# tokkiwa/FlashGMM

Hardware: AMD Instinct MI355X
Metric: encode+decode Mpixels/s (Kodak, K=4 N=192) + GMM-CDF HBM GB/s vs roofline (higher is better)
Workload: dtype f32; 1 GPU; kodak24; schedule=codec, images_per_gpu=24, K=4, approx_mode=polya, param_dtype=f32, coded_symbols_per_gpu=6223104, streams_per_gpu=48, one_device_rehearsal=False

## Files before the change

### flashgmm_amd/csrc/fgmm_capi.cpp

```cpp
#include <sched.h>

#include <string>

#include "fgmm_ctx.h"

using namespace fgmm;

namespace fgmm {

static thread_local char t_err[512] = "";
char *last_error_buffer(size_t *cap) {
  if (cap) *cap = sizeof t_err;
  return t_err;
}
int fail(int code, const char *fmt, ...) {
  va_list ap;
  va_start(ap, fmt);
  vsnprintf(t_err, sizeof t_err, fmt, ap);
  va_end(ap);
  return code;
}

}

// ... 123 lines not shown
  const char *name;
  int64_t fgmm_ctx::Opts::*field;
  int64_t lo, hi;
  const char *env;
};
const OptName kOpts[] = {
    {"pieces", &fgmm_ctx::Opts::pieces, 0, kMaxPieces, "FGMM_PIECES"},
    {"dec_first", &fgmm_ctx::Opts::dec_first, 1, 1 << 20, "FGMM_DEC_FIRST"},
    {"tab_cap_e", &fgmm_ctx::Opts::tab_cap_e, 256, 32768, "FGMM_TAB_CAP_E"},
    {"stage_max_mb", &fgmm_ctx::Opts::stage_max_mb, 0, 1 << 30, "FGMM_STAGE_MAX_MB"},
    {"trace", &fgmm_ctx::Opts::trace, 0, 2, "FGMM_TRACE"},
    {"enc_vec", &fgmm_ctx::Opts::enc_vec, 0, 8, "FGMM_VEC"},
    {"enc_linear", &fgmm_ctx::Opts::enc_linear, 0, 1, nullptr},
    {"ef_rows", &fgmm_ctx::Opts::ef_rows, 0, 2, "FGMM_EF_ROWS"},
    {"ef_min", &fgmm_ctx::Opts::ef_min, kTabEfMin, 1 << 20, "FGMM_EF_MIN_ROWS"},
    {"enc_ways", &fgmm_ctx::Opts::enc_ways, 0, kMaxEncWays, "FGMM_ENC_WAYS"},
    {"ckpt_decode", &fgmm_ctx::Opts::ckpt_decode, 0, 2, "FGMM_CKPT_DECODE"},
    {"spin_lat", &fgmm_ctx::Opts::spin_lat, -1, 1ll << 40, "FGMM_SPIN_LAT"},
    {"gpu_decode", &fgmm_ctx::Opts::gpu_decode, 0, 2, "FGMM_GPU_DECODE"},
    {"enc_segs", &fgmm_ctx::Opts::enc_segs, 0, 2, "FGMM_ENC_SEGS"},
    {"scatter_rounds", &fgmm_ctx::Opts::scatter_rounds, 0, 1, nullptr},
};
}

namespace {
double cgroup_cpu_quota() {
  double best = -1.0;
  auto take = [&best](double q) {
    if (q > 0 && (best < 0 || q < best)) best = q;
  };
// ... 727 lines not shown
  hd->meta = reinterpret_cast<uint32_t *>(ctx->d_ws + 1024);
  dev::Stream s = (dev::Stream)stream;
  DEV_TRY(dev::copy_async(ctx->d_ws, hd, sizeof *hd, dev::kH2D, s));
  DEV_TRY(dev::memset_async(ctx->d_ws + 1024, 0, meta_bytes, s));
  LAUNCH_TRY(launch_symtab(reinterpret_cast<const EncDesc *>(ctx->d_ws), 1, 1, n, n, false, mode, enc_vec4_ok(*hd, false) ? 4 : 1, false, false, s));
  DEV_TRY(dev::stream_sync(s));
  return FGMM_OK;
}

int fgmm_build_cdftab_hip(fgmm_ctx *ctx, void *stream, const float *scales, const float *means,
                          const float *weights, int64_t n, int64_t stride_n, int64_t stride_k, int mode,
                          int32_t max_bs, int flags, uint32_t *hdr, uint8_t *pool, uint64_t pool_cap,
                          uint64_t *pool_used) {
  if (!ctx || n < 0 || !mode_ok(mode) || !pool_used) return fail(FGMM_ERR_INVALID, "bad argument");
  if (max_bs < 0 || max_bs > FGMM_MAX_BS_H4) return fail(FGMM_ERR_UNSUPPORTED, "max_bs %d outside [0, %d] (4-byte headers)", max_bs, FGMM_MAX_BS_H4);
  std::lock_guard<std::mutex> lock(ctx->mu);
  DeviceGuard g(ctx->device);
  const int32_t tiles = (int32_t)((n + 255) / 256);
  const size_t o_bsum = 2048, o_boff = o_bsum + align_up(sizeof(uint32_t) * (size_t)tiles + 64, 256);
  int rc;
  if ((rc = ctx->ensure_device(o_boff + sizeof(uint64_t) * (size_t)tiles + 64)) || (rc = ctx->ensure_host(4096))) return rc;
  dev::Stream s = (dev::Stream)stream;
  DecDesc *hd = reinterpret_cast<DecDesc *>(ctx->h_ws);
  memset(hd, 0, sizeof *hd);
  hd->scales = scales;
  hd->means = means;
  hd->weights = weights;
  hd->stride_k = stride_k;
  hd->stride_p = stride_n;
  hd->hw = n;
// ... 42 lines not shown
  dev::Stream s = (dev::Stream)stream;
  DecDesc *hd = reinterpret_cast<DecDesc *>(ctx->h_ws);
  memset(hd, 0, sizeof *hd);
  hd->scales = scales;
  hd->means = means;
  hd->weights = weights;
  hd->stride_k = stride_k;
  hd->stride_p = stride_n;
  hd->hw = n;
  hd->n = n;
  hd->n_ch = 1;
  hd->max_bs = max_bs;
  hd->prune = (flags & FGMM_TAB_NO_PRUNE) ? 0 : 1;
  hd->clamp = (flags & FGMM_TAB_CLAMP) ? 1 : 0;
  hd->hdr_form = tab_hdr_form(max_bs);
  hd->ef_min = (flags & FGMM_TAB_RAW_ROWS) ? kTabNoEf : kTabEfMin;
  hd->tl = tl;
  hd->blk_begin = 0;
  hd->blk_end = (int32_t)nblk;
  hd->hdr_out = hdr;
  hd->blkoff_out = blk_off;
  hd->rows = rows;
  hd->rows_cap = rows_cap;
  hd->counters = reinterpret_cast<unsigned long long *>(ctx->d_ws + 1024);
  hd->count_edges = 1;
  unsigned long long cn[kTabCounters] = {};
  DEV_TRY(dev::copy_async(ctx->d_ws, hd, sizeof *hd, dev::kH2D, s));
  DEV_TRY(dev::memset_async(ctx->d_ws + 1024, 0, kCounterBytes, s));
  if (n) LAUNCH_TRY(launch_tab(reinterpret_cast<const DecDesc *>(ctx->d_ws), 1, (int)nblk, tl, cap_e, mode, (flags & FGMM_TAB_CLAMP) != 0, false, s));
  DEV_TRY(dev::copy_async(cn, ctx->d_ws + 1024, sizeof cn, dev::kD2H, s));
  DEV_TRY(dev::stream_sync(s));
// ... 63 lines not shown
```

### flashgmm_amd/csrc/fgmm_ctx.h

```cpp
#pragma once
#include <math.h>
#include <pthread.h>
#include <sched.h>
#include <stdarg.h>
#include <stdio.h>
#include <stdlib.h>
#include <string.h>

#include <algorithm>
#include <atomic>
#include <chrono>
#include <condition_variable>
#include <functional>
#include <mutex>
#include <queue>
#include <string>
#include <thread>
#include <vector>

#include "../../include/flashgmm_amd.h"
#include "fgmm_device.h"
#include "fgmm_internal.h"

namespace fgmm {
// ... 267 lines not shown
  std::mutex mu;
  fgmm::Pool *pool = nullptr;
  fgmm::WorkerCpus worker_cpus;
  fgmm::Pool *dec_pool = nullptr;
  fgmm::Pool *decoders() const { return dec_pool ? dec_pool : pool; }
  char *d_ws = nullptr;
  size_t d_cap = 0;
  char *h_ws = nullptr;
  size_t h_cap = 0;
  std::vector<fgmm::dev::Event> events;
  std::vector<fgmm::dev::Event> sleep_events;
  fgmm::dev::Stream copy_stream = nullptr;
  fgmm::dev::Stream aux_stream = nullptr;
  struct Opts {
    int64_t pieces = 0, dec_first = 2, tab_cap_e = fgmm::kTabCapE, stage_max_mb = 0, trace = 0, enc_vec = 0, enc_linear = 1, ef_rows = 0,
            ef_min = fgmm::kTabEfDefault, enc_ways = 0, ckpt_decode = 0, spin_lat = 400000, gpu_decode = 0, enc_segs = 1, scatter_rounds = 1;
  } opt;
  struct Chunk {
    char *p;
    size_t cap, used;
  };
  std::vector<Chunk> chunks;
  void chunks_reset() {
    for (auto &c : chunks) c.used = 0;
  }
  int chunk_alloc(size_t bytes, char **out);
  char *d_stage = nullptr;
  size_t d_stage_cap = 0;
  int ensure_stage(size_t bytes);
  size_t stage_budget() const;
  int ensure_streams();
// ... 103 lines not shown
```

### flashgmm_amd/csrc/fgmm_decode.cpp

```cpp
#include <array>

#include "fgmm_ctx.h"

namespace fgmm {
namespace {

struct Part {
  int item;
  int64_t blk_begin, blk_end;
  size_t o_hdr, o_blkoff;
  int piece;
};
struct Unit {
  std::vector<Part> parts;
  size_t fixed = 0, rows_cap = 0;
  size_t o_stage = 0;
  char *d_range = nullptr;
};
struct Key {
  int unit, item, seg;
  bool operator>(const Key &o) const { return unit != o.unit ? unit > o.unit : (item != o.item ? item > o.item : seg > o.seg); }
};

constexpr int kLaunchAhead = 3;

struct DecodeCall {
  fgmm_ctx *ctx;
  dev::Stream stream;
  std::vector<DecItem> &items;
  const int mode, count;
  Trace tr;
  int cap_e = kTabCapE, np = 1, decoders = 1;
  bool clamped = false, f16 = false, spin = false;
  uint32_t ef_min = kTabNoEf;
  int64_t streams_of_work = 0;
  bool lead_small = false;
  double lead_cum[kMaxPieces + 1] = {0};
  std::vector<int> fast, generic;
  std::vector<Unit> units;
  int n_units = 0;
  Arena ar;
  size_t o_descs = 0, o_scat = 0, o_counters = 0, upload_bytes = 0, stage_total = 0, n_parts = 0;
  std::vector<size_t> unit_desc0;
  int n_round = 0, M_round = 0;
  int64_t hw_round = 0;
  bool dead_round = false;
  dev::Event *ev_kernel = nullptr, *ev_counters = nullptr, *ev_landed = nullptr;
  TempDevice temp;
  int launched = 0;
// ... 20 lines not shown
    if (ctx->opt.tab_cap_e == kTabCapE)
      for (const DecItem &it : items)
        if (!tab_tl(it.max_bs, cap_e) && tab_tl(it.max_bs, kTabCapEWide)) {
          cap_e = kTabCapEWide;
          break;
        }
    clamped = items[0].clamp != 0;
    f16 = items[0].prm.dtype == FGMM_F16;
    const bool use_ckpt = ctx->opt.ckpt_decode == 1 || (ctx->opt.ckpt_decode == 0 && count < std::max(ctx->decoders()->size(), 1));
    for (auto &it : items) {
      if (!use_ckpt) it.ckpt = nullptr, it.n_ckpt = 0;
      streams_of_work += it.ckpt && it.n_ckpt > 0 ? it.n_ckpt + 1 : 1;
    }
    decoders = (int)std::min<int64_t>(std::max(ctx->decoders()->size(), 1), streams_of_work);
    ef_min = ctx->opt.ef_rows == 1 || (ctx->opt.ef_rows == 0 && decoders >= 10) ? (uint32_t)ctx->opt.ef_min : kTabNoEf;
    return FGMM_OK;
  }

  int plan_items() {
    for (int i = 0; i < count; ++i) {
      DecItem &it = items[i];
      if (it.max_bs < 0 || it.max_bs > FGMM_MAX_BS) return fail(FGMM_ERR_UNSUPPORTED, "max_bs_value %d outside [0, %d]", it.max_bs, FGMM_MAX_BS);
      it.n_ch = 0;
      for (int c = 0; c < it.M; ++c) it.n_ch += it.zero_bitmap ? (it.zero_bitmap[c] != 0) : 1;
      it.n = (int64_t)it.n_ch * it.hw;
      it.o_list = ar.take(sizeof(int32_t) * std::max(it.n_ch, 1), 16);
      it.o_rank = ar.take(sizeof(int32_t) * std::max(it.M, 1), 16);
      it.hdr_form = tab_hdr_form(it.max_bs);
      it.ef_min = ef_min;
      it.tl = tab_tl(it.max_bs, cap_e);
      it.nblk = it.tl ? (it.n + it.tl - 1) / it.tl : 0;
      if (it.nblk > 0x7FFFFFFFll) it.tl = 0, it.nblk = 0;
      (it.tl ? fast : generic).push_back(i);
    }
    return FGMM_OK;
  }

  void plan_pieces() {
    np = (int)std::min<int64_t>(std::max<int64_t>(ctx->opt.pieces, 1), kMaxPieces);
    int64_t lat = 0, lat_max = 0;
    for (int i : fast) lat += items[i].n, lat_max = std::max(lat_max, items[i].n);
    if (ctx->opt.pieces > 0) return;
    np = 8;
    while (np < kAutoPiecesMax && (int64_t)np * (np + 1) / 2 * 4096 < lat_max) ++np;
    if (lat < 65536) np = 1;
    if (decoders == 1 && np > 1) {
      lead_small = true;
// ... 141 lines not shown
    d.scales = it.prm.scales;
    d.means = it.prm.means;
    d.weights = it.prm.weights;
    d.stride_k = it.prm.stride_k;
    d.stride_c = it.prm.stride_c;
    d.stride_p = it.stride_p;
    d.hw = it.hw;
    d.n = it.n;
    d.chan_list = reinterpret_cast<const int32_t *>(ctx->d_ws + it.o_list);
    d.n_ch = it.n_ch;
    d.max_bs = it.max_bs;
    d.clamp = it.clamp;
    d.logits = (it.prm.flags & FGMM_PARAMS_LOGITS) ? 1 : 0;
    d.prune = 1;
    d.hdr_form = it.hdr_form;
    d.ef_min = ef_min;
    d.tl = it.tl;
    d.count_edges = ctx->profiling ? 1 : 0;
    return d;
  }
  void fill_unit_descs(int u) {
    const Unit &un = units[(size_t)u];
    DecDesc *hd = reinterpret_cast<DecDesc *>(ctx->h_ws + o_descs);
    for (size_t k = 0; k < un.parts.size(); ++k) {
      const Part &p = un.parts[k];
      DecDesc &d = hd[unit_desc0[(size_t)u] + k];
      d = base_desc(items[p.item]);
      d.blk_begin = (int32_t)p.blk_begin;
      d.blk_end = (int32_t)p.blk_end;
      d.hdr_out = un.d_range + p.o_hdr;
      d.blkoff_out = reinterpret_cast<uint32_t *>(un.d_range + p.o_blkoff);
// ... 526 lines not shown
```

### flashgmm_amd/csrc/fgmm_internal.h

```cpp
#pragma once
#include <stddef.h>
#include <stdint.h>

#include "../../include/flashgmm_amd.h"

#if defined(__HIPCC__)
#define FGMM_HD __host__ __device__
#else
#define FGMM_HD
#endif

namespace fgmm {


struct EncDesc {
  const float *y;
  const int32_t *sym;
  const void *scales, *means, *weights;
  int64_t stride_k, stride_c, stride_p;
  int64_t hw;
  int32_t M;
  int32_t clamp;
  int32_t logits;
  uint32_t meta_slots;
// ... 120 lines not shown
FGMM_HD static inline uint32_t tab_hdr_cnt(uint32_t h) { return (h >> 16) & 0x7FFFu; }
FGMM_HD static inline uint32_t tab_hdr_nonmono(uint32_t h) { return h >> 31; }
FGMM_HD static inline unsigned long long tab_hdr8_pack(int32_t a, uint32_t cnt, uint32_t nonmono) {
  return (unsigned long long)(uint32_t)a | ((unsigned long long)((cnt & 0x7FFFFFFFu) | (nonmono << 31)) << 32);
}
constexpr uint32_t kTabNoEf = 0x7FFFFFFFu;
FGMM_HD static inline bool tab_row_is_ef(uint32_t cnt, uint32_t nonmono, uint32_t ef_min) { return cnt >= ef_min && !nonmono; }
constexpr uint32_t kTabEf12Max = 48;
FGMM_HD static inline uint32_t tab_ef_l(uint32_t cnt) { return cnt <= kTabEf12Max ? 12u : 8u; }
FGMM_HD static inline uint32_t tab_ef_hb(uint32_t cnt, uint32_t l) { return cnt + (65536u >> l); }
FGMM_HD static inline uint32_t tab_ef_lb(uint32_t cnt, uint32_t l) { return (tab_ef_hb(cnt, l) + 7u) & ~7u; }
FGMM_HD static inline unsigned long long tab_ef_bits(uint32_t cnt, uint32_t l) { return (unsigned long long)cnt * l + tab_ef_lb(cnt, l); }
FGMM_HD static inline unsigned long long tab_row_bytes(uint32_t cnt, uint32_t nonmono, uint32_t ef_min) {
  return tab_row_is_ef(cnt, nonmono, ef_min) ? 2ull * ((tab_ef_bits(cnt, tab_ef_l(cnt)) + 15ull) >> 4) : 2ull * (unsigned long long)cnt;
}
FGMM_HD static inline bool tab_hdr_fits16(int32_t max_bs) { return 2 * (int64_t)max_bs + 2 <= 254; }
FGMM_HD static inline int tab_hdr_form(int32_t max_bs) { return tab_hdr_fits16(max_bs) ? 2 : (max_bs <= 16382 ? 4 : 8); }
constexpr int kTabCapE = 12288;
constexpr int kTabCapEWide = 16384;
constexpr int kTabMaxTl = 256;
FGMM_HD static inline int tab_tl(int32_t max_bs, int cap_e) {
  const int64_t W = 2 * (int64_t)max_bs + 2;
  const int64_t t = (cap_e / W) & ~15ll;
  return t >= 16 ? (int)(t > kTabMaxTl ? kTabMaxTl : t) : 0;
}

int launch_quant_stats(const EncDesc *d_descs, int count, int M_max, void *stream);
int launch_symtab(const EncDesc *d_descs, int count, int M_max, int64_t hw_max, int64_t n_max, bool linear, int mode, int vec,
                  bool clamped, bool f16, void *stream);
int launch_cdf_pair(const int32_t *v, const float *scales, const float *means, const float *weights, int64_t n,
// ... 86 lines not shown
```

### flashgmm_amd/csrc/fgmm_rans.cpp

```cpp
#include <immintrin.h>
#include <stdlib.h>
#include <string.h>

#include <cmath>
#include <mutex>
#include <vector>

#include "../../include/flashgmm_amd.h"
#include "fgmm_internal.h"

namespace fgmm {

namespace {

constexpr uint64_t kRansL = 1ull << 31;
constexpr uint32_t kPrec = 16;
constexpr uint32_t kMaxCdf = 65535;
constexpr uint32_t kBypassBits = 4;
constexpr uint32_t kMaxBypassVal = 15;

struct Rcp {
  uint64_t rcp;
  uint32_t shift;
  uint32_t bias_add;
// ... 494 lines not shown
      const int64_t rem = (int64_t)nbits - 64 * (int64_t)w;
      if (rem < 64) m &= (1ull << rem) - 1ull;
      if (m) break;
      if (__builtin_expect(++w >= r.words(), 0)) return -1;
      m = r[w];
    }
    const int32_t pos = w * 64 + (int32_t)__builtin_ctzll(m);
    e1 = ((uint32_t)(pos - j) << r.l) | r.low(j);
  }
  *jout = j;
  *start = e0;
  *freq = (e1 - e0) & 0xFFFFu;
  return 1;
}

}

int TabDecoder::begin(const uint8_t *enc, size_t enc_len, const TabView *view, int64_t n_, int32_t max_bs_, int32_t *out_) {
  tv = view;
  n = n_;
  max_bs = max_bs_;
  out = out_;
  i = 0;
  next_piece = 0;
  rc = FGMM_OK;
  copy = nullptr;
  scratch = nullptr;
  scratch_cap = 0;
  if (n < 0 || !enc || (n > 0 && (!out || !tv || !tv->piece || tv->npiece < 1))) return rc = FGMM_ERR_INVALID;
  if (tv && tv->hdr_form != 2 && tv->hdr_form != 4 && tv->hdr_form != 8) return rc = FGMM_ERR_INVALID;
// ... 97 lines not shown
        uint32_t h;
        memcpy(&h, rowp, 4);
        rowp += 4;
        cnt = tab_hdr_cnt(h);
        nonmono = tab_hdr_nonmono(h);
      }
    } else if (hdr_form == 4) {
      const uint32_t h = static_cast<const uint32_t *>(pc->hdr)[li];
      cnt = tab_hdr_cnt(h);
      nonmono = tab_hdr_nonmono(h);
    } else {
      const uint64_t h = static_cast<const uint64_t *>(pc->hdr)[li];
      cnt = (int64_t)((h >> 32) & 0x7FFFFFFFu);
      nonmono = (uint32_t)(h >> 63);
    }
    const uint64_t rbytes = tab_row_bytes((uint32_t)cnt, nonmono, ef_min);
    if (cnt < 1 || (uint64_t)(rows_end - rowp) < rbytes) { rc = FGMM_ERR_INVALID; return; }
    rowp += rbytes;
    ++i;
  }
  inline bool active() const { return rc == FGMM_OK && i < i_end; }
  void finish() {
    td->x = dec.x;
    td->ptr = dec.ptr;
    td->i = i;
    if (rc != FGMM_OK) td->rc = rc;
  }

  inline void open_block() {
    b_end = i + tl < i_end ? i + tl : i_end;
    if (pc->blk_off) {
      rowp = pc->rows + 4 * (size_t)pc->blk_off[blk];
      if (__builtin_expect(rowp > rows_end, 0)) {
        rc = FGMM_ERR_INVALID;
        return;
      }
      if (b_end < i_end) {
        const uint8_t *nx = pc->rows + 4 * (size_t)pc->blk_off[blk + 1];
        if (nx + FGMM_PREFETCH_AHEAD <= rows_end)
          for (int q = 0; q < FGMM_PREFETCH_AHEAD; q += 64) __builtin_prefetch(nx + q);
      }
    }
    ++blk;
  }

  __attribute__((always_inline)) inline void step() {
    if (__builtin_expect(i == b_end, 0)) {
      open_block();
      if (rc != FGMM_OK) return;
    }
    __builtin_prefetch(rowp + FGMM_PREFETCH_AHEAD);
    __builtin_prefetch(rowp + FGMM_PREFETCH_AHEAD + 64);
    int64_t a;
    int64_t cnt;
    uint32_t nonmono;
    const int64_t li = i - i_beg;
    if (hdr_form == 2) {
      const uint32_t c = static_cast<const uint16_t *>(pc->hdr)[li];
      a = (int64_t)(c & 0xFFu) - max_bs;
      cnt = c >> 8;
      nonmono = 0;
      if (__builtin_expect(cnt == kHdr2Escape, 0)) {
        if (rows_end - rowp < 4) { rc = FGMM_ERR_INVALID; return; }
        uint32_t h;
        memcpy(&h, rowp, 4);
        rowp += 4;
        a = tab_hdr_a(h);
        cnt = tab_hdr_cnt(h);
        nonmono = tab_hdr_nonmono(h);
      }
    } else if (hdr_form == 4) {
      const uint32_t h = static_cast<const uint32_t *>(pc->hdr)[li];
      a = tab_hdr_a(h);
      cnt = tab_hdr_cnt(h);
      nonmono = tab_hdr_nonmono(h);
    } else {
      const uint64_t h = static_cast<const uint64_t *>(pc->hdr)[li];
      a = (int32_t)(uint32_t)h;
      cnt = (int64_t)((h >> 32) & 0x7FFFFFFFu);
      nonmono = (uint32_t)(h >> 63);
    }
    if (__builtin_expect(cnt < 1 || a < -(int64_t)max_bs || a + max_bs + cnt > W, 0)) { rc = FGMM_ERR_INVALID; return; }
    const bool is_ef = tab_row_is_ef((uint32_t)cnt, nonmono, ef_min);
    const uint64_t rbytes = tab_row_bytes((uint32_t)cnt, nonmono, ef_min);
    if (__builtin_expect((uint64_t)(rows_end - rowp) < rbytes, 0)) { rc = FGMM_ERR_INVALID; return; }
    const bool zero_before = a > -(int64_t)max_bs;
    const uint8_t *row_bytes = rowp;
    rowp += rbytes;

    const uint32_t cf = (uint32_t)(dec.x & 0xFFFFu);
    int32_t value;
    if (__builtin_expect(cf == kMaxCdf, 0)) {
      value = dec.bypass();
    } else {
      uint32_t start = 0, freq = 0;
      bool done = false;
      if (!is_ef) {
        const uint16_t *row = reinterpret_cast<const uint16_t *>(row_bytes);
        if (__builtin_expect(!nonmono, 1)) {
          const int32_t j = upper_bound_u16(row, (int32_t)cnt, cf);
          if (__builtin_expect(j >= 1 && j < cnt, 1)) {
            start = row[j - 1];
            freq = (uint32_t)(row[j] - start) & 0xFFFFu;
            value = (int32_t)(a + j - 1);
            done = true;
          } else if (j == 0 && zero_before) {
            start = 0;
            freq = row[0];
            value = (int32_t)(a - 1);
            done = true;
          }
        }
// ... 9 lines not shown
          rc = FGMM_ERR_INVALID;
          return;
        } else {
          value = expand_and_bisect(r, a, cf, &start, &freq);
          if (rc != FGMM_OK) return;
        }
      }
      if (__builtin_expect(freq == 0, 0)) { rc = FGMM_ERR_INVALID; return; }
      dec.advance(start, freq);
    }
    td->out[i] = value;
    if (__builtin_expect(dec.underrun, 0)) { rc = FGMM_ERR_STREAM; return; }
    ++i;
  }

  __attribute__((noinline)) int32_t expand_and_bisect(const EfRow &r, int64_t a, uint32_t cf, uint32_t *start, uint32_t *freq) {
    const int32_t cnt = r.cnt;
    if ((size_t)cnt > td->scratch_cap) {
      free(td->scratch);
      td->scratch_cap = (size_t)cnt + 64;
      td->scratch = (uint16_t *)malloc(td->scratch_cap * sizeof(uint16_t));
      if (!td->scratch) {
        td->scratch_cap = 0;
        rc = FGMM_ERR_NOMEM;
        return 0;
      }
    }
    for (int32_t q = 0; q < cnt; ++q) {
      const int32_t pos = ef_select1(r, (uint32_t)q);
      if (pos < q) {
        rc = FGMM_ERR_INVALID;
        return 0;
      }
      td->scratch[q] = (uint16_t)((((uint32_t)(pos - q)) << r.l) | r.low(q));
    }
    return bisect_reference(Row{td->scratch, (int32_t)a, cnt}, cf, max_bs, start, freq);
  }
};

}

int TabDecoder::piece(int k) {
  PieceRun r;
  if (!r.begin(*this, k)) return r.rc;
  while (r.active()) r.step();
  r.finish();
  return rc;
}

int TabDecoder::segment(int64_t lo, int64_t hi, uint64_t x0, uint64_t pos0, uint64_t *x1, uint64_t *pos1) {
  if (rc != FGMM_OK) return rc;
  if (!tv || lo < 0 || hi > n || lo > hi || pos0 > (uint64_t)(end_ - base_)) return rc = FGMM_ERR_INVALID;
  x = x0;
  ptr = base_ + pos0;
  i = lo;
  int k = 0;
  while (k < tv->npiece && tv->piece[k].end <= lo) ++k;
  for (; i < hi && k < tv->npiece && rc == FGMM_OK; ++k) {
    PieceRun r;
    if (!r.begin_at(*this, k, hi)) {
      if (r.rc != FGMM_OK) rc = r.rc;
      break;
    }
    while (r.active()) r.step();
    r.finish();
  }
  if (rc == FGMM_OK && i < hi) rc = FGMM_ERR_INVALID;
  *x1 = x;
  *pos1 = (uint64_t)(ptr - base_);
  return rc;
}

int TabDecoder::finish() {
  if (rc == FGMM_OK && i < n) rc = FGMM_ERR_INVALID;
  free(copy);
  free(scratch);
  copy = nullptr;
  scratch = nullptr;
  return rc;
// ... 218 lines not shown
                                 size_t *out_len, fgmm_ckpt *ckpt_out) {
  if (stride < 0 || (stride & (stride - 1))) return FGMM_ERR_INVALID;
  return fgmm::rans_encode_symtab_ckpt(packed, symbols_or_null, n, -1, out, out_len, stride, ckpt_out);
}
int fgmm_rans_decode_tab_ckpt(const uint8_t *encoded, size_t encoded_len, const void *hdr, int hdr_form, const uint32_t *blk_off,
                              int32_t tl, const uint8_t *rows, uint64_t rows_len, int64_t n, int32_t max_bs, int flags,
                              const fgmm_ckpt *ckpt, int64_t n_ckpt, int64_t stride, int32_t *out_symbols, int32_t *verified_out) {
  if (verified_out) *verified_out = 0;
  if (!ckpt || n_ckpt == 0 || !blk_off || stride <= 0 || (stride & (stride - 1)) || n_ckpt != fgmm_ckpt_count(n, stride))
    return fgmm_rans_decode_tab(encoded, encoded_len, hdr, hdr_form, blk_off, tl, rows, rows_len, n, max_bs, flags, out_symbols);
  if (n > 0 && (!hdr || !rows)) return FGMM_ERR_INVALID;
  if (max_bs < 0 || max_bs > FGMM_MAX_BS || tl < 1) return FGMM_ERR_INVALID;
  if (hdr_form == 2 && !fgmm::tab_hdr_fits16(max_bs)) return FGMM_ERR_INVALID;
  if (hdr_form == 4 && max_bs > FGMM_MAX_BS_H4) return FGMM_ERR_INVALID;
  const fgmm::TabPiece pc{hdr, blk_off, rows, (size_t)rows_len, n};
  const fgmm::TabView tv{(flags & FGMM_TAB_RAW_ROWS) ? fgmm::kTabNoEf : fgmm::kTabEfMin, hdr_form, tl, 1, &pc, nullptr, nullptr};
  bool ok = true;
  int hard = FGMM_OK;
  fgmm::TabDecoder td;
  int rc = td.begin(encoded, encoded_len, &tv, n, max_bs, out_symbols);
  if (rc != FGMM_OK) {
    td.finish();
    return rc;
  }
  const uint64_t x_head = td.x;
  for (int64_t sgm = 0; sgm <= n_ckpt && ok; ++sgm) {
    const int64_t lo = sgm * stride, hi = sgm == n_ckpt ? n : (sgm + 1) * stride;
    const uint64_t x0 = sgm ? ckpt[sgm - 1].x : x_head, pos0 = sgm ? ckpt[sgm - 1].pos : 0;
    uint64_t x1 = 0, pos1 = 0;
    rc = td.segment(lo, hi, x0, pos0, &x1, &pos1);
    td.rc = FGMM_OK;
// ... 48 lines not shown
  for (int k = 0; k < ways; ++k) {
    syms[k] = symbols_or_null ? symbols_or_null[k] : nullptr;
    nb[k] = -1;
    out[k] = nullptr;
    o[k] = &out[k];
    l[k] = &out_len[k];
  }
  return fgmm::rans_encode_symtab_ways(ways, packed, syms, n, nb, o, l);
}

int fgmm_rans_decode_cdftab(const uint8_t *encoded, size_t encoded_len, const uint32_t *hdr, const uint8_t *pool,
                            uint64_t pool_len, int64_t n, int32_t max_bs, int flags, int32_t *out_symbols) {
  if (n > 0 && (!hdr || !pool)) return FGMM_ERR_INVALID;
  if (max_bs < 0 || max_bs > FGMM_MAX_BS_H4) return FGMM_ERR_UNSUPPORTED;
  const fgmm::TabPiece pc{hdr, nullptr, pool, (size_t)pool_len, n};
  const fgmm::TabView tv{(flags & FGMM_TAB_RAW_ROWS) ? fgmm::kTabNoEf : fgmm::kTabEfMin, 4, 0, 1, &pc, nullptr, nullptr};
  return fgmm::rans_decode_tab(encoded, encoded_len, tv, n, max_bs, out_symbols);
}

int fgmm_rans_decode_tab(const uint8_t *encoded, size_t encoded_len, const void *hdr, int hdr_form, const uint32_t *blk_off,
                         int32_t tl, const uint8_t *rows, uint64_t rows_len, int64_t n, int32_t max_bs, int flags,
                         int32_t *out_symbols) {
  if (n > 0 && (!hdr || !rows)) return FGMM_ERR_INVALID;
  if (max_bs < 0 || max_bs > FGMM_MAX_BS || (blk_off && tl < 1)) return FGMM_ERR_INVALID;
  if (hdr_form == 2 && !fgmm::tab_hdr_fits16(max_bs)) return FGMM_ERR_INVALID;
  if (hdr_form == 4 && max_bs > FGMM_MAX_BS_H4) return FGMM_ERR_INVALID;
  const fgmm::TabPiece pc{hdr, blk_off, rows, (size_t)rows_len, n};
  const fgmm::TabView tv{(flags & FGMM_TAB_RAW_ROWS) ? fgmm::kTabNoEf : fgmm::kTabEfMin, hdr_form, tl, 1, &pc, nullptr, nullptr};
  return fgmm::rans_decode_tab(encoded, encoded_len, tv, n, max_bs, out_symbols);
}

void fgmm_free(void *p) { free(p); }

struct fgmm_symbuf {
  fgmm::SymBuf sb;
};
struct fgmm_decstream {
  fgmm::DecStream ds;
};

int fgmm_symbuf_create(fgmm_symbuf **out) {
  if (!out) return FGMM_ERR_INVALID;
  *out = new (std::nothrow) fgmm_symbuf;
// ... 60 lines not shown
```

### flashgmm_amd/csrc/fgmm_tab.hip

```cpp
#include <algorithm>

#include "fgmm_dev.h"

namespace fgmm {

template <int MODE, bool CLAMPED, typename PT> struct TabLatent {
  float mu[4], sg[4], pi[4], rs[4];
  int max_bs;

  __device__ __forceinline__ void load(const DecDesc &d, int c, int64_t p) {
    const int64_t base = (int64_t)c * d.stride_c + p * d.stride_p;
#pragma unroll
    for (int k = 0; k < 4; ++k) {
      const float s = ld1<PT>(d.scales, base + k * d.stride_k);
      sg[k] = CLAMPED ? clamp_scale(s) : s;
      rs[k] = CLAMPED ? rcp_refined(sg[k]) : 0.0f;
      mu[k] = ld1<PT>(d.means, base + k * d.stride_k);
      pi[k] = ld1<PT>(d.weights, base + k * d.stride_k);
    }
    if (d.logits) softmax4(pi);
    max_bs = d.max_bs;
  }
  __device__ __forceinline__ uint32_t edge(int j) const {
    const float x = (float)(j - max_bs) - 0.5f;
// ... 429 lines not shown
      for (int q = 0; q < 8; ++q) v[q] = e32[(k >> 1) + q];
#pragma unroll
      for (int q = 0; q < 8; ++q) {
        ts.step(j_lo + k + 2 * q, v[q] & 0xFFFFu);
        ts.step(j_lo + k + 2 * q + 1, v[q] >> 16);
      }
    }
    for (; k < len; ++k) ts.step(j_lo + k, e[k]);
    int a_idx;
    uint32_t cnt;
    ts.finish(j_hi, W, S.tsat[tid], a_idx, cnt);
    const uint32_t nm = ts.nonmono ? 1u : 0u;
    S.meta[tid] = (uint32_t)a_idx | (cnt << 16);
    if (nm) S.flags[tid] |= 2;
    bytes = (uint32_t)tab_row_bytes(cnt, nm, d.ef_min);
    const int64_t li = (int64_t)(b - d.blk_begin) * tl + tid;
    if (d.hdr_form == 2) {
      const uint32_t c8 = nm ? kHdr2Escape : cnt;
      static_cast<uint16_t *>(d.hdr_out)[li] = (uint16_t)((uint32_t)a_idx | (c8 << 8));
      if (nm) bytes += 4;
    } else if (d.hdr_form == 4) {
      static_cast<uint32_t *>(d.hdr_out)[li] = tab_hdr_pack(a_idx - max_bs, cnt, nm);
    } else {
      static_cast<unsigned long long *>(d.hdr_out)[li] = tab_hdr8_pack(a_idx - max_bs, cnt, nm);
    }
  }
  TAB_T(2);
  uint32_t B, EFT;
  const uint32_t exB = tab_scan(bytes, S.scratch, &B);
  const uint32_t B4 = (B + 3u) & ~3u;
// ... 19 lines not shown
    S.scratch[10] = fits ? 1u : 0u;
    if (d.count_edges) atomicAdd(&d.counters[4 + (b & (kTabEdgeSlots - 1))], 2ull * NP);
  }
  for (uint32_t q = tid; q < (EFT >> 16); q += kBlock) S.bitmap[q] = 0;
  {
    const int any_nm = __syncthreads_or(tid < nl && (S.flags[tid] & 2));
    if (tid == 0 && any_nm) atomicAdd(&d.counters[3], 1ull);
  }
  if (!S.scratch[10]) return;

  struct RowRef {
    const uint16_t *e;
    int j_lo, j_hi, a_idx;
    uint32_t cnt, nm, T_sat, aux;
    uint32_t efl, HB, LB, M;
    __device__ __forceinline__ void load(const TabSmem &S, const uint16_t *E16, int l, uint32_t ef_min) {
      const uint32_t w = S.win[l], mt = S.meta[l];
      j_lo = (int)(w & 0xFFFFu);
      j_hi = j_lo + (int)(w >> 16);
      a_idx = (int)(mt & 0xFFFFu);
      cnt = mt >> 16;
      nm = (S.flags[l] >> 1) & 1u;
      T_sat = S.tsat[l];
      e = E16 + 2 * (size_t)S.offP[l] - j_lo;
      aux = S.efoff[l];
      efl = tab_row_is_ef(cnt, nm, ef_min) ? tab_ef_l(cnt) : 0u;
      HB = efl ? tab_ef_hb(cnt, efl) : 0u;
      LB = (HB + 7u) & ~7u;
      M = efl == 8u ? (1u << 20) / 8u + 1u : (efl == 12u ? (1u << 20) / 12u + 1u : (efl ? (1u << 20) / efl + 1u : 0u));
    }
    __device__ __forceinline__ uint32_t entry(uint32_t k) const {
      const int idx = a_idx + (int)k;
      return idx < j_lo ? 0u : (idx >= j_hi ? T_sat : (uint32_t)e[idx]);
    }
  };

  TAB_T(3);
  {
    const uint32_t NE = EFT & 0xFFFFu;
    const uint32_t per = (NE + kBlock - 1u) / kBlock;
    uint32_t t = (uint32_t)tid * per;
    const uint32_t t_end = std::min(NE, t + per);
    if (t < t_end) {
// ... 37 lines not shown
    const uint32_t per = (NW + kBlock - 1u) / kBlock;
    uint32_t q = (uint32_t)tid * per;
    const uint32_t q_end = std::min(NW, q + per);
    int l = 0;
    uint32_t r_beg = 0, r_end = 0;
    RowRef R;
    if (q < q_end) {
      l = find_owner(S.rowoff, nl, 4 * q);
      r_beg = S.rowoff[l];
      r_end = S.rowoff[l + 1];
      R.load(S, E16, l, d.ef_min);
    }
    auto unit = [&](uint32_t h) -> uint32_t {
      const bool escaped = d.hdr_form == 2 && R.nm;
      if (escaped && h < 2) return (tab_hdr_pack(R.a_idx - max_bs, R.cnt, 1u) >> (16 * h)) & 0xFFFFu;
      if (!R.efl) return R.entry(escaped ? h - 2 : h);
      const uint32_t bit0 = 16 * h;
      uint32_t v = 0;
      if (bit0 < R.HB) v = (S.bitmap[(R.aux >> 16) + (h >> 1)] >> (16 * (h & 1u))) & 0xFFFFu;
      if (bit0 + 16 > R.LB) {
        const int rel = (int)bit0 - (int)R.LB;
        uint32_t j = rel > 0 ? ((uint32_t)rel * R.M) >> 20 : 0u;
        const uint32_t mask = (1u << R.efl) - 1u;
        for (; j < R.cnt; ++j) {
          const int sh = (int)(j * R.efl) - rel;
          if (sh >= 16) break;
          const uint32_t lowbits = R.entry(j) & mask;
          v |= sh >= 0 ? lowbits << sh : lowbits >> -sh;
        }
        v &= 0xFFFFu;
// ... 573 lines not shown
```

### include/flashgmm_amd.h

```cpp
#ifndef FLASHGMM_AMD_H
#define FLASHGMM_AMD_H

#include <stddef.h>
#include <stdint.h>

#ifdef __cplusplus
extern "C" {
#endif

#define FGMM_ABI_VERSION 6

typedef enum {
  FGMM_OK = 0,
  FGMM_ERR_INVALID = 1,
  FGMM_ERR_NO_DEVICE = 2,
  FGMM_ERR_HIP = 3,
  FGMM_ERR_NOMEM = 4,
  FGMM_ERR_STREAM = 5,
  FGMM_ERR_UNSUPPORTED = 6
} fgmm_status;

typedef enum { FGMM_MODE_POLYA = 0, FGMM_MODE_AS = 1, FGMM_MODE_LOGISTIC = 2 } fgmm_mode;

typedef enum { FGMM_HOST = 0, FGMM_DEVICE = 1 } fgmm_memspace;
// ... 110 lines not shown


int fgmm_gmm_cdf_hip(fgmm_ctx *ctx, void *stream, const int32_t *v, const float *scales, const float *means,
                     const float *weights, int64_t n, int64_t stride_n, int64_t stride_k, int mode, float *c1,
                     float *c2);

int fgmm_softmax4_hip(fgmm_ctx *ctx, void *stream, const float *logits, float *weights, int64_t n);

int fgmm_build_symtab_hip(fgmm_ctx *ctx, void *stream, const int32_t *symbols, const float *scales,
                          const float *means, const float *weights, int64_t n, int64_t stride_n, int64_t stride_k,
                          int mode, uint32_t *packed);

#define FGMM_TAB_NO_PRUNE 1
#define FGMM_TAB_CLAMP 2
#define FGMM_TAB_RAW_ROWS 4
#define FGMM_HDR_FORM(max_bs) ((2 * (int64_t)(max_bs) + 2 <= 254) ? 2 : ((max_bs) <= FGMM_MAX_BS_H4 ? 4 : 8))
int fgmm_build_cdftab_hip(fgmm_ctx *ctx, void *stream, const float *scales, const float *means,
                          const float *weights, int64_t n, int64_t stride_n, int64_t stride_k, int mode,
                          int32_t max_bs, int flags, uint32_t *hdr, uint8_t *pool, uint64_t pool_cap,
                          uint64_t *pool_used);
int fgmm_build_tab_hip(fgmm_ctx *ctx, void *stream, const float *scales, const float *means, const float *weights,
                       int64_t n, int64_t stride_n, int64_t stride_k, int mode, int32_t max_bs, int flags, void *hdr,
                       uint32_t *blk_off, uint8_t *rows, uint64_t rows_cap, uint64_t *rows_used, int32_t *tl_out);

int fgmm_selftest_saturation(fgmm_ctx *ctx, int mode, uint64_t *n_bad_out);

int fgmm_selftest_fastmath(fgmm_ctx *ctx, int which, uint64_t n, uint64_t seed, uint64_t *n_bad_out);

int fgmm_rans_encode_symtab(const uint32_t *packed, const int32_t *symbols_or_null, int64_t n, uint8_t **out,
                            size_t *out_len);
// ... 61 lines not shown
```

Before: 1063 Mpixels/s.

## Add grouped delta-coded CDF table rows with per-group bit widths

```diff
diff --git a/flashgmm_amd/csrc/fgmm_capi.cpp b/flashgmm_amd/csrc/fgmm_capi.cpp
--- a/flashgmm_amd/csrc/fgmm_capi.cpp
+++ b/flashgmm_amd/csrc/fgmm_capi.cpp
@@ -161,6 +161,8 @@
     {"enc_linear", &fgmm_ctx::Opts::enc_linear, 0, 1, nullptr},
     {"ef_rows", &fgmm_ctx::Opts::ef_rows, 0, 2, "FGMM_EF_ROWS"},
     {"ef_min", &fgmm_ctx::Opts::ef_min, kTabEfMin, 1 << 20, "FGMM_EF_MIN_ROWS"},
+    {"grp_rows", &fgmm_ctx::Opts::grp_rows, 0, 2, "FGMM_GRP_ROWS"},
+    {"grp_min", &fgmm_ctx::Opts::grp_min, 17, 1 << 20, "FGMM_GRP_MIN_ROWS"},
     {"enc_ways", &fgmm_ctx::Opts::enc_ways, 0, kMaxEncWays, "FGMM_ENC_WAYS"},
     {"ckpt_decode", &fgmm_ctx::Opts::ckpt_decode, 0, 2, "FGMM_CKPT_DECODE"},
     {"spin_lat", &fgmm_ctx::Opts::spin_lat, -1, 1ll << 40, "FGMM_SPIN_LAT"},
@@ -918,6 +920,7 @@
                           uint64_t *pool_used) {
   if (!ctx || n < 0 || !mode_ok(mode) || !pool_used) return fail(FGMM_ERR_INVALID, "bad argument");
   if (max_bs < 0 || max_bs > FGMM_MAX_BS_H4) return fail(FGMM_ERR_UNSUPPORTED, "max_bs %d outside [0, %d] (4-byte headers)", max_bs, FGMM_MAX_BS_H4);
+  if (flags & FGMM_TAB_GROUPED) return fail(FGMM_ERR_UNSUPPORTED, "FGMM_TAB_GROUPED: the generic kernels do not write grouped rows");
   std::lock_guard<std::mutex> lock(ctx->mu);
   DeviceGuard g(ctx->device);
   const int32_t tiles = (int32_t)((n + 255) / 256);
@@ -990,7 +993,7 @@
   hd->prune = (flags & FGMM_TAB_NO_PRUNE) ? 0 : 1;
   hd->clamp = (flags & FGMM_TAB_CLAMP) ? 1 : 0;
   hd->hdr_form = tab_hdr_form(max_bs);
-  hd->ef_min = (flags & FGMM_TAB_RAW_ROWS) ? kTabNoEf : kTabEfMin;
+  hd->ef_min = (flags & FGMM_TAB_GROUPED) ? (kTabGrouped | kGrpMinDefault) : (flags & FGMM_TAB_RAW_ROWS) ? kTabNoEf : kTabEfMin;
   hd->tl = tl;
   hd->blk_begin = 0;
   hd->blk_end = (int32_t)nblk;
diff --git a/flashgmm_amd/csrc/fgmm_ctx.h b/flashgmm_amd/csrc/fgmm_ctx.h
--- a/flashgmm_amd/csrc/fgmm_ctx.h
+++ b/flashgmm_amd/csrc/fgmm_ctx.h
@@ -305,7 +305,8 @@
   fgmm::dev::Stream aux_stream = nullptr;
   struct Opts {
     int64_t pieces = 0, dec_first = 2, tab_cap_e = fgmm::kTabCapE, stage_max_mb = 0, trace = 0, enc_vec = 0, enc_linear = 1, ef_rows = 0,
-            ef_min = fgmm::kTabEfDefault, enc_ways = 0, ckpt_decode = 0, spin_lat = 400000, gpu_decode = 0, enc_segs = 1, scatter_rounds = 1;
+            ef_min = fgmm::kTabEfDefault, enc_ways = 0, ckpt_decode = 0, spin_lat = 400000, gpu_decode = 0, enc_segs = 1, scatter_rounds = 1,
+            grp_rows = 2, grp_min = fgmm::kGrpMinDefault;
   } opt;
   struct Chunk {
     char *p;
diff --git a/flashgmm_amd/csrc/fgmm_decode.cpp b/flashgmm_amd/csrc/fgmm_decode.cpp
--- a/flashgmm_amd/csrc/fgmm_decode.cpp
+++ b/flashgmm_amd/csrc/fgmm_decode.cpp
@@ -33,6 +33,7 @@
   int cap_e = kTabCapE, np = 1, decoders = 1;
   bool clamped = false, f16 = false, spin = false;
   uint32_t ef_min = kTabNoEf;
+  uint32_t grp_min = 0;
   int64_t streams_of_work = 0;
   bool lead_small = false;
   double lead_cum[kMaxPieces + 1] = {0};
@@ -83,6 +84,7 @@
     }
     decoders = (int)std::min<int64_t>(std::max(ctx->decoders()->size(), 1), streams_of_work);
     ef_min = ctx->opt.ef_rows == 1 || (ctx->opt.ef_rows == 0 && decoders >= 10) ? (uint32_t)ctx->opt.ef_min : kTabNoEf;
+    grp_min = ctx->opt.grp_rows == 1 || (ctx->opt.grp_rows == 0 && ef_min != kTabNoEf) ? (kTabGrouped | (uint32_t)ctx->opt.grp_min) : 0u;
     return FGMM_OK;
   }
 
@@ -96,10 +98,10 @@
       it.o_list = ar.take(sizeof(int32_t) * std::max(it.n_ch, 1), 16);
       it.o_rank = ar.take(sizeof(int32_t) * std::max(it.M, 1), 16);
       it.hdr_form = tab_hdr_form(it.max_bs);
-      it.ef_min = ef_min;
       it.tl = tab_tl(it.max_bs, cap_e);
       it.nblk = it.tl ? (it.n + it.tl - 1) / it.tl : 0;
       if (it.nblk > 0x7FFFFFFFll) it.tl = 0, it.nblk = 0;
+      it.ef_min = it.tl && grp_min ? grp_min : ef_min;
       (it.tl ? fast : generic).push_back(i);
     }
     return FGMM_OK;
@@ -271,7 +273,7 @@
     d.logits = (it.prm.flags & FGMM_PARAMS_LOGITS) ? 1 : 0;
     d.prune = 1;
     d.hdr_form = it.hdr_form;
-    d.ef_min = ef_min;
+    d.ef_min = it.ef_min;
     d.tl = it.tl;
     d.count_edges = ctx->profiling ? 1 : 0;
     return d;
diff --git a/flashgmm_amd/csrc/fgmm_internal.h b/flashgmm_amd/csrc/fgmm_internal.h
--- a/flashgmm_amd/csrc/fgmm_internal.h
+++ b/flashgmm_amd/csrc/fgmm_internal.h
@@ -158,6 +158,22 @@
 FGMM_HD static inline unsigned long long tab_row_bytes(uint32_t cnt, uint32_t nonmono, uint32_t ef_min) {
   return tab_row_is_ef(cnt, nonmono, ef_min) ? 2ull * ((tab_ef_bits(cnt, tab_ef_l(cnt)) + 15ull) >> 4) : 2ull * (unsigned long long)cnt;
 }
+constexpr uint32_t kTabGrouped = 0x80000000u;
+constexpr uint32_t kGrpG = 8;
+constexpr uint32_t kGrpMinDefault = 33;
+FGMM_HD static inline bool tab_grouped(uint32_t ef_min) { return (ef_min >> 31) != 0; }
+FGMM_HD static inline bool tab_row_is_grp(uint32_t cnt, uint32_t nonmono, uint32_t ef_min) {
+  return tab_grouped(ef_min) && cnt >= (ef_min & 0x7FFFFFFFu) && !nonmono;
+}
+FGMM_HD static inline uint32_t tab_grp_ns(uint32_t cnt) { return (cnt + kGrpG - 1u) / kGrpG; }
+FGMM_HD static inline uint32_t tab_grp_wu(uint32_t ns) { return (ns + 3u) >> 2; }
+FGMM_HD static inline uint32_t tab_grp_klast(uint32_t cnt) { return cnt - 1u - kGrpG * (tab_grp_ns(cnt) - 1u); }
+FGMM_HD static inline uint32_t tab_grp_code(uint32_t maxdiff) {
+  uint32_t w = 0;
+  while (maxdiff >> w) ++w;
+  return w >= 15u ? 15u : w;
+}
+FGMM_HD static inline uint32_t tab_grp_width(uint32_t code) { return code < 15u ? code : 16u; }
 FGMM_HD static inline bool tab_hdr_fits16(int32_t max_bs) { return 2 * (int64_t)max_bs + 2 <= 254; }
 FGMM_HD static inline int tab_hdr_form(int32_t max_bs) { return tab_hdr_fits16(max_bs) ? 2 : (max_bs <= 16382 ? 4 : 8); }
 constexpr int kTabCapE = 12288;
diff --git a/flashgmm_amd/csrc/fgmm_rans.cpp b/flashgmm_amd/csrc/fgmm_rans.cpp
--- a/flashgmm_amd/csrc/fgmm_rans.cpp
+++ b/flashgmm_amd/csrc/fgmm_rans.cpp
@@ -532,6 +532,108 @@
   return 1;
 }
 
+__attribute__((target("popcnt"))) inline uint32_t grp_nib_sum(uint64_t x) {
+  const uint64_t f = x & (x >> 1) & (x >> 2) & (x >> 3) & 0x1111111111111111ull;
+  const uint64_t b = (x & 0x0F0F0F0F0F0F0F0Full) + ((x >> 4) & 0x0F0F0F0F0F0F0F0Full);
+  return (uint32_t)((b * 0x0101010101010101ull) >> 56) + (uint32_t)__builtin_popcountll(f);
+}
+struct GrpRow {
+  const uint16_t *samp;
+  const uint8_t *wid;
+  const uint8_t *bits;
+  int32_t cnt, ns, klast;
+  inline uint32_t width(int32_t g) const { return tab_grp_width((uint32_t)(wid[g >> 1] >> (4 * (g & 1))) & 15u); }
+  __attribute__((target("popcnt"))) inline uint32_t wsum(int32_t g) const {
+    uint32_t s = 0;
+    const uint8_t *p = wid;
+    uint64_t x;
+    for (; g >= 16; g -= 16, p += 8) {
+      memcpy(&x, p, 8);
+      s += grp_nib_sum(x);
+    }
+    memcpy(&x, p, 8);
+    return s + grp_nib_sum(x & ((1ull << (4 * g)) - 1ull));
+  }
+  inline bool expand(int32_t g, uint32_t bit0, uint32_t (&e)[8], int32_t *k_out) const {
+    const int32_t k = g == ns - 1 ? klast : 7;
+    const uint32_t w = width(g), mask = (1u << w) - 1u;
+    unsigned __int128 v;
+    memcpy(&v, bits + (bit0 >> 3), 16);
+    v >>= (bit0 & 7u);
+    uint32_t acc = samp[g];
+    e[0] = acc;
+#pragma GCC unroll 7
+    for (int32_t q = 0; q < 7; ++q) {
+      acc += (uint32_t)(v >> (q * w)) & mask & (0u - (uint32_t)(q < k));
+      e[q + 1] = acc;
+    }
+    *k_out = k;
+    return acc <= 0xFFFFu;
+  }
+};
+inline bool grp_open(const uint8_t *p, uint64_t avail, int64_t cnt, GrpRow *r, uint64_t *rbytes) {
+  if (avail < 2) return false;
+  uint16_t L;
+  memcpy(&L, p, 2);
+  const uint32_t ns = tab_grp_ns((uint32_t)cnt), wu = tab_grp_wu(ns);
+  *rbytes = 2ull * L;
+  if ((uint64_t)L < 1ull + ns + wu || avail < 2ull * L) return false;
+  r->samp = reinterpret_cast<const uint16_t *>(p) + 1;
+  r->wid = p + 2 * (1 + (size_t)ns);
+  r->bits = r->wid + 2 * (size_t)wu;
+  r->cnt = (int32_t)cnt;
+  r->ns = (int32_t)ns;
+  r->klast = (int32_t)tab_grp_klast((uint32_t)cnt);
+  const uint64_t nbits = 7ull * r->wsum((int32_t)ns - 1) + (uint64_t)r->klast * r->width((int32_t)ns - 1);
+  return ((nbits + 15) >> 4) == (uint64_t)L - 1 - ns - wu;
+}
+__attribute__((target("avx2,popcnt"))) inline int grp_bracket(const GrpRow &r, uint32_t cf, bool zero_before, int32_t *jout, uint32_t *start,
+                                                              uint32_t *freq) {
+  const int32_t js = upper_bound_u16(r.samp, r.ns, cf);
+  if (__builtin_expect(js == 0, 0)) {
+    if (!zero_before) return 0;
+    *jout = 0, *start = 0, *freq = r.samp[0];
+    return 1;
+  }
+  const int32_t g = js - 1;
+  uint32_t e[8];
+  int32_t k;
+  if (__builtin_expect(!r.expand(g, 7u * r.wsum(g), e, &k), 0)) return -1;
+  int32_t c = 0;
+#pragma GCC unroll 8
+  for (int32_t q = 0; q < 8; ++q) c += (int32_t)(e[q] <= cf) & (int32_t)(q <= k);
+  uint32_t hi;
+  if (c <= k) {
+    hi = e[c];
+  } else if (js < r.ns) {
+    hi = r.samp[js];
+    if (__builtin_expect(hi < e[k], 0)) return -1;
+  } else {
+    return 0;
+  }
+  *jout = 8 * g + c;
+  *start = e[c - 1];
+  *freq = hi - e[c - 1];
+  return 1;
+}
+inline bool grp_expand_row(const GrpRow &r, uint16_t *out) {
+  uint32_t bit0 = 0, prev = 0;
+  for (int32_t g = 0; g < r.ns; ++g) {
+    uint32_t e[8];
+    int32_t k;
+    if (!r.expand(g, bit0, e, &k) || e[0] < prev) return false;
+    for (int32_t q = 0; q <= k; ++q) out[8 * g + q] = (uint16_t)e[q];
+    prev = e[k];
+    bit0 += (uint32_t)k * r.width(g);
+  }
+  return true;
+}
+
+}
+
+static inline uint32_t tab_flags_ef_min(int flags) {
+  if (flags & FGMM_TAB_GROUPED) return fgmm::kTabGrouped | fgmm::kGrpMinDefault;
+  return (flags & FGMM_TAB_RAW_ROWS) ? fgmm::kTabNoEf : fgmm::kTabEfMin;
 }
 
 int TabDecoder::begin(const uint8_t *enc, size_t enc_len, const TabView *view, int64_t n_, int32_t max_bs_, int32_t *out_) {
@@ -659,7 +761,14 @@
       cnt = (int64_t)((h >> 32) & 0x7FFFFFFFu);
       nonmono = (uint32_t)(h >> 63);
     }
-    const uint64_t rbytes = tab_row_bytes((uint32_t)cnt, nonmono, ef_min);
+    uint64_t rbytes = tab_row_bytes((uint32_t)cnt, nonmono, ef_min);
+    if (tab_row_is_grp((uint32_t)cnt, nonmono, ef_min)) {
+      if (rows_end - rowp < 2) { rc = FGMM_ERR_INVALID; return; }
+      uint16_t L;
+      memcpy(&L, rowp, 2);
+      rbytes = 2ull * L;
+      if (L < 1) { rc = FGMM_ERR_INVALID; return; }
+    }
     if (cnt < 1 || (uint64_t)(rows_end - rowp) < rbytes) { rc = FGMM_ERR_INVALID; return; }
     rowp += rbytes;
     ++i;
@@ -689,7 +798,7 @@
     ++blk;
   }
 
-  __attribute__((always_inline)) inline void step() {
+  template <int HF, int LONG> __attribute__((always_inline)) inline void step() {
     if (__builtin_expect(i == b_end, 0)) {
       open_block();
       if (rc != FGMM_OK) return;
@@ -700,7 +809,7 @@
     int64_t cnt;
     uint32_t nonmono;
     const int64_t li = i - i_beg;
-    if (hdr_form == 2) {
+    if (HF == 2) {
       const uint32_t c = static_cast<const uint16_t *>(pc->hdr)[li];
       a = (int64_t)(c & 0xFFu) - max_bs;
       cnt = c >> 8;
@@ -714,7 +823,7 @@
         cnt = tab_hdr_cnt(h);
         nonmono = tab_hdr_nonmono(h);
       }
-    } else if (hdr_form == 4) {
+    } else if (HF == 4) {
       const uint32_t h = static_cast<const uint32_t *>(pc->hdr)[li];
       a = tab_hdr_a(h);
       cnt = tab_hdr_cnt(h);
@@ -726,9 +835,13 @@
       nonmono = (uint32_t)(h >> 63);
     }
     if (__builtin_expect(cnt < 1 || a < -(int64_t)max_bs || a + max_bs + cnt > W, 0)) { rc = FGMM_ERR_INVALID; return; }
-    const bool is_ef = tab_row_is_ef((uint32_t)cnt, nonmono, ef_min);
-    const uint64_t rbytes = tab_row_bytes((uint32_t)cnt, nonmono, ef_min);
-    if (__builtin_expect((uint64_t)(rows_end - rowp) < rbytes, 0)) { rc = FGMM_ERR_INVALID; return; }
+    const bool is_ef = LONG == 1 && tab_row_is_ef((uint32_t)cnt, nonmono, ef_min);
+    const bool is_grp = LONG == 2 && tab_row_is_grp((uint32_t)cnt, nonmono, ef_min);
+    uint64_t rbytes = LONG == 1 ? tab_row_bytes((uint32_t)cnt, nonmono, ef_min) : 2ull * (uint64_t)cnt;
+    GrpRow gr;
+    if (is_grp) {
+      if (__builtin_expect(!grp_open(rowp, (uint64_t)(rows_end - rowp), cnt, &gr, &rbytes), 0)) { rc = FGMM_ERR_INVALID; return; }
+    } else if (__builtin_expect((uint64_t)(rows_end - rowp) < rbytes, 0)) { rc = FGMM_ERR_INVALID; return; }
     const bool zero_before = a > -(int64_t)max_bs;
     const uint8_t *row_bytes = rowp;
     rowp += rbytes;
@@ -740,7 +853,19 @@
     } else {
       uint32_t start = 0, freq = 0;
       bool done = false;
-      if (!is_ef) {
+      if (is_grp) {
+        int32_t j;
+        const int br = grp_bracket(gr, cf, zero_before, &j, &start, &freq);
+        if (__builtin_expect(br > 0, 1)) {
+          value = (int32_t)(a + j - 1);
+        } else if (br < 0) {
+          rc = FGMM_ERR_INVALID;
+          return;
+        } else {
+          value = expand_and_bisect_grp(gr, a, cf, &start, &freq);
+          if (rc != FGMM_OK) return;
+        }
+      } else if (!is_ef) {
         const uint16_t *row = reinterpret_cast<const uint16_t *>(row_bytes);
         if (__builtin_expect(!nonmono, 1)) {
           const int32_t j = upper_bound_u16(row, (int32_t)cnt, cf);
@@ -780,8 +905,18 @@
     ++i;
   }
 
-  __attribute__((noinline)) int32_t expand_and_bisect(const EfRow &r, int64_t a, uint32_t cf, uint32_t *start, uint32_t *freq) {
-    const int32_t cnt = r.cnt;
+  template <int HF> inline void run_hf() {
+    if (tab_grouped(ef_min)) while (active()) step<HF, 2>();
+    else if (ef_min == kTabNoEf) while (active()) step<HF, 0>();
+    else while (active()) step<HF, 1>();
+  }
+  void run() {
+    if (hdr_form == 2) run_hf<2>();
+    else if (hdr_form == 4) run_hf<4>();
+    else run_hf<8>();
+  }
+
+  bool scratch_for(int32_t cnt) {
     if ((size_t)cnt > td->scratch_cap) {
       free(td->scratch);
       td->scratch_cap = (size_t)cnt + 64;
@@ -789,9 +924,23 @@
       if (!td->scratch) {
         td->scratch_cap = 0;
         rc = FGMM_ERR_NOMEM;
-        return 0;
+        return false;
       }
     }
+    return true;
+  }
+  __attribute__((noinline)) int32_t expand_and_bisect_grp(const GrpRow &r, int64_t a, uint32_t cf, uint32_t *start, uint32_t *freq) {
+    if (!scratch_for(r.cnt + 8)) return 0;
+    if (!grp_expand_row(r, td->scratch)) {
+      rc = FGMM_ERR_INVALID;
+      return 0;
+    }
+    return bisect_reference(Row{td->scratch, (int32_t)a, r.cnt}, cf, max_bs, start, freq);
+  }
+
+  __attribute__((noinline)) int32_t expand_and_bisect(const EfRow &r, int64_t a, uint32_t cf, uint32_t *start, uint32_t *freq) {
+    const int32_t cnt = r.cnt;
+    if (!scratch_for(cnt)) return 0;
     for (int32_t q = 0; q < cnt; ++q) {
       const int32_t pos = ef_select1(r, (uint32_t)q);
       if (pos < q) {
@@ -809,7 +958,7 @@
 int TabDecoder::piece(int k) {
   PieceRun r;
   if (!r.begin(*this, k)) return r.rc;
-  while (r.active()) r.step();
+  r.run();
   r.finish();
   return rc;
 }
@@ -828,7 +977,7 @@
       if (r.rc != FGMM_OK) rc = r.rc;
       break;
     }
-    while (r.active()) r.step();
+    r.run();
     r.finish();
   }
   if (rc == FGMM_OK && i < hi) rc = FGMM_ERR_INVALID;
@@ -1077,7 +1226,7 @@
   if (hdr_form == 2 && !fgmm::tab_hdr_fits16(max_bs)) return FGMM_ERR_INVALID;
   if (hdr_form == 4 && max_bs > FGMM_MAX_BS_H4) return FGMM_ERR_INVALID;
   const fgmm::TabPiece pc{hdr, blk_off, rows, (size_t)rows_len, n};
-  const fgmm::TabView tv{(flags & FGMM_TAB_RAW_ROWS) ? fgmm::kTabNoEf : fgmm::kTabEfMin, hdr_form, tl, 1, &pc, nullptr, nullptr};
+  const fgmm::TabView tv{fgmm::tab_flags_ef_min(flags), hdr_form, tl, 1, &pc, nullptr, nullptr};
   bool ok = true;
   int hard = FGMM_OK;
   fgmm::TabDecoder td;
@@ -1156,7 +1305,7 @@
   if (n > 0 && (!hdr || !pool)) return FGMM_ERR_INVALID;
   if (max_bs < 0 || max_bs > FGMM_MAX_BS_H4) return FGMM_ERR_UNSUPPORTED;
   const fgmm::TabPiece pc{hdr, nullptr, pool, (size_t)pool_len, n};
-  const fgmm::TabView tv{(flags & FGMM_TAB_RAW_ROWS) ? fgmm::kTabNoEf : fgmm::kTabEfMin, 4, 0, 1, &pc, nullptr, nullptr};
+  const fgmm::TabView tv{fgmm::tab_flags_ef_min(flags), 4, 0, 1, &pc, nullptr, nullptr};
   return fgmm::rans_decode_tab(encoded, encoded_len, tv, n, max_bs, out_symbols);
 }
 
@@ -1168,7 +1317,7 @@
   if (hdr_form == 2 && !fgmm::tab_hdr_fits16(max_bs)) return FGMM_ERR_INVALID;
   if (hdr_form == 4 && max_bs > FGMM_MAX_BS_H4) return FGMM_ERR_INVALID;
   const fgmm::TabPiece pc{hdr, blk_off, rows, (size_t)rows_len, n};
-  const fgmm::TabView tv{(flags & FGMM_TAB_RAW_ROWS) ? fgmm::kTabNoEf : fgmm::kTabEfMin, hdr_form, tl, 1, &pc, nullptr, nullptr};
+  const fgmm::TabView tv{fgmm::tab_flags_ef_min(flags), hdr_form, tl, 1, &pc, nullptr, nullptr};
   return fgmm::rans_decode_tab(encoded, encoded_len, tv, n, max_bs, out_symbols);
 }
 
diff --git a/flashgmm_amd/csrc/fgmm_tab.hip b/flashgmm_amd/csrc/fgmm_tab.hip
--- a/flashgmm_amd/csrc/fgmm_tab.hip
+++ b/flashgmm_amd/csrc/fgmm_tab.hip
@@ -467,6 +467,29 @@
     S.meta[tid] = (uint32_t)a_idx | (cnt << 16);
     if (nm) S.flags[tid] |= 2;
     bytes = (uint32_t)tab_row_bytes(cnt, nm, d.ef_min);
+    if (tab_row_is_grp(cnt, nm, d.ef_min)) {
+      uint8_t *gw = reinterpret_cast<uint8_t *>(S.bitmap + (S.offP[tid] >> 4) + 2u * (uint32_t)tid);
+      const uint32_t T_sat = S.tsat[tid];
+      auto ent = [&](uint32_t q) -> uint32_t {
+        const int idx = a_idx + (int)q;
+        return idx < j_lo ? 0u : (idx >= j_hi ? T_sat : (uint32_t)e[idx - j_lo]);
+      };
+      const uint32_t ns = tab_grp_ns(cnt);
+      uint32_t bits = 0;
+      for (uint32_t g = 0; g < ns; ++g) {
+        const uint32_t q0 = kGrpG * g, kk = std::min(kGrpG - 1u, cnt - 1u - q0);
+        uint32_t prev = ent(q0), mx = 0;
+        for (uint32_t q = 1; q <= kk; ++q) {
+          const uint32_t cur = ent(q0 + q);
+          mx = std::max(mx, cur - prev);
+          prev = cur;
+        }
+        const uint32_t code = mx ? std::min(32u - (uint32_t)__clz(mx), 15u) : 0u;
+        gw[g] = (uint8_t)code;
+        bits += kk * tab_grp_width(code);
+      }
+      bytes = 2u * (1u + ns + tab_grp_wu(ns) + ((bits + 15u) >> 4));
+    }
     const int64_t li = (int64_t)(b - d.blk_begin) * tl + tid;
     if (d.hdr_form == 2) {
       const uint32_t c8 = nm ? kHdr2Escape : cnt;
@@ -516,6 +539,8 @@
     int j_lo, j_hi, a_idx;
     uint32_t cnt, nm, T_sat, aux;
     uint32_t efl, HB, LB, M;
+    uint32_t gns;
+    const uint8_t *gw;
     __device__ __forceinline__ void load(const TabSmem &S, const uint16_t *E16, int l, uint32_t ef_min) {
       const uint32_t w = S.win[l], mt = S.meta[l];
       j_lo = (int)(w & 0xFFFFu);
@@ -529,6 +554,8 @@
       efl = tab_row_is_ef(cnt, nm, ef_min) ? tab_ef_l(cnt) : 0u;
       HB = efl ? tab_ef_hb(cnt, efl) : 0u;
       LB = (HB + 7u) & ~7u;
+      gns = tab_row_is_grp(cnt, nm, ef_min) ? tab_grp_ns(cnt) : 0u;
+      gw = reinterpret_cast<const uint8_t *>(S.bitmap + (S.offP[l] >> 4) + 2u * (uint32_t)l);
       M = efl == 8u ? (1u << 20) / 8u + 1u : (efl == 12u ? (1u << 20) / 12u + 1u : (efl ? (1u << 20) / efl + 1u : 0u));
     }
     __device__ __forceinline__ uint32_t entry(uint32_t k) const {
@@ -596,6 +623,36 @@
     auto unit = [&](uint32_t h) -> uint32_t {
       const bool escaped = d.hdr_form == 2 && R.nm;
       if (escaped && h < 2) return (tab_hdr_pack(R.a_idx - max_bs, R.cnt, 1u) >> (16 * h)) & 0xFFFFu;
+      if (R.gns) {
+        const uint32_t ns = R.gns, wu = tab_grp_wu(ns);
+        if (h == 0) return (r_end - r_beg) >> 1;
+        if (h <= ns) return R.entry(kGrpG * (h - 1u));
+        if (h <= ns + wu) {
+          const uint32_t g0 = 4u * (h - 1u - ns);
+          uint32_t v = 0;
+          for (uint32_t t = 0; t < 4u && g0 + t < ns; ++t) v |= (uint32_t)R.gw[g0 + t] << (4u * t);
+          return v;
+        }
+        const uint32_t bit0 = 16u * (h - 1u - ns - wu);
+        uint32_t v = 0, pos = 0;
+        for (uint32_t g = 0; g < ns && pos < bit0 + 16u; ++g) {
+          const uint32_t w = tab_grp_width(R.gw[g]), q0 = kGrpG * g, kk = std::min(kGrpG - 1u, R.cnt - 1u - q0);
+          const uint32_t next = pos + kk * w;
+          if (next > bit0) {
+            uint32_t q = pos < bit0 ? (bit0 - pos) / w : 0u;
+            uint32_t prev = R.entry(q0 + q);
+            for (; q < kk; ++q) {
+              const int sh = (int)(pos + q * w) - (int)bit0;
+              if (sh >= 16) break;
+              const uint32_t cur = R.entry(q0 + q + 1u), dlt = cur - prev;
+              prev = cur;
+              v |= sh >= 0 ? dlt << sh : dlt >> -sh;
+            }
+          }
+          pos = next;
+        }
+        return v & 0xFFFFu;
+      }
       if (!R.efl) return R.entry(escaped ? h - 2 : h);
       const uint32_t bit0 = 16 * h;
       uint32_t v = 0;
diff --git a/include/flashgmm_amd.h b/include/flashgmm_amd.h
--- a/include/flashgmm_amd.h
+++ b/include/flashgmm_amd.h
@@ -148,6 +148,7 @@
 #define FGMM_TAB_NO_PRUNE 1
 #define FGMM_TAB_CLAMP 2
 #define FGMM_TAB_RAW_ROWS 4
+#define FGMM_TAB_GROUPED 8
 #define FGMM_HDR_FORM(max_bs) ((2 * (int64_t)(max_bs) + 2 <= 254) ? 2 : ((max_bs) <= FGMM_MAX_BS_H4 ? 4 : 8))
 int fgmm_build_cdftab_hip(fgmm_ctx *ctx, void *stream, const float *scales, const float *means,
                           const float *weights, int64_t n, int64_t stride_n, int64_t stride_k, int mode,
```

Measured after the change: 944.0 Mpixels/s. 11.2% lower.
